# bowang-lab/BioReason

Hardware: AMD Instinct MI355X
Metric: GRPO samples/sec (NT-500M+Qwen3-1.7B, DNA 2x1024, prompt 2180, gen 256) (higher is better)
Workload: dtype bf16

## Files before the change

bioreason_amd/csrc/k_misc.hip:

```cpp
#include "bra_device.h"
#include "bra_api_internal.h"

namespace bra {

template <int HD>
__global__ __launch_bounds__(256) void head_transpose_kernel(const bf16_t* x, long sb, long ss, long sh, bf16_t* xt,
                                                             long t_sb, long t_sh, long pitch, int S) {
    constexpr int LD = HD + 2;
    __shared__ bf16_t tile[64 * LD];
    const int tid = (int)threadIdx.x;
    const int s0 = (int)blockIdx.x * 64, h = (int)blockIdx.y, b = (int)blockIdx.z;
    const bf16_t* xp = x + b * sb + h * sh;
    constexpr int CH = HD / 8;
    for (int q = tid; q < 64 * CH; q += 256) {
        const int r = q / CH, c = q % CH;
        const int s = s0 + r;
        u32x4 v = {0u, 0u, 0u, 0u};
        if (s < S) v = ld16(xp + (long)s * ss + c * 8);
        uint32_t* tp = reinterpret_cast<uint32_t*>(&tile[r * LD + c * 8]);
        tp[0] = v.x; tp[1] = v.y; tp[2] = v.z; tp[3] = v.w;
    }
    __syncthreads();
    bf16_t* op = xt + b * t_sb + h * t_sh;
    for (int q = tid; q < HD * 8; q += 256) {
        const int d = q >> 3, c = q & 7;
        uint32_t w[4];
#pragma unroll
        for (int i = 0; i < 4; ++i) {
            const uint32_t lo = tile[(c * 8 + 2 * i) * LD + d], hi = tile[(c * 8 + 2 * i + 1) * LD + d];
            w[i] = lo | (hi << 16);
        }
        u32x4 v = {w[0], w[1], w[2], w[3]};
        st16(op + (long)d * pitch + s0 + c * 8, v);
    }
}

__global__ __launch_bounds__(256) void attn_delta_kernel(const bf16_t* dout, long do_sb, long do_ss, long do_sh,
                                                         const bf16_t* o, long o_sb, long o_ss, long o_sh,
                                                         float* delta, int B, int S, int H, int hd) {
    const int lpr = hd / 8;
    const long total = (long)B * H * S * lpr;
    const long idx = (long)blockIdx.x * 256 + threadIdx.x;
    const bool live = idx < total;
    const long cl = live ? idx : total - 1;
    const int c = (int)(cl % lpr);
    const long row = cl / lpr;
    const int s = (int)(row % S);
    const int h = (int)((row / S) % H);
    const int b = (int)(row / ((long)S * H));
    float f[8], g[8];
    unpack8(ld16(dout + b * do_sb + (long)s * do_ss + h * do_sh + c * 8), f);
    unpack8(ld16(o + b * o_sb + (long)s * o_ss + h * o_sh + c * 8), g);
    float acc = 0.f;
#pragma unroll
    for (int i = 0; i < 8; ++i) acc += f[i] * g[i];
    for (int m = lpr >> 1; m >= 1; m >>= 1) acc += wave_shfl_xor(acc, m);
    if (live && c == 0) delta[row] = acc;
}

__global__ __launch_bounds__(1024) void dna_scatter_plan_kernel(const int* ids, int ntok, int dna_id,
                                                                const uint8_t* dna_mask, int nseq, int Sd,
                                                                const int* seq_order, int* tok_src, int* counts) {
    __shared__ int feat_base[1025];
    __shared__ int wsum[16];
    __shared__ int carry;
    const int tid = (int)threadIdx.x, lane = tid & 63, wave = tid >> 6;
    for (int k = wave; k < nseq; k += 16) {
        const int seq = seq_order[k];
        int cnt = 0;
        for (int p = lane; p < Sd; p += 64) cnt += dna_mask[(long)seq * Sd + p] ? 1 : 0;
        for (int m = 32; m >= 1; m >>= 1) cnt += wave_shfl_xor_i(cnt, m);
        if (lane == 0) feat_base[k + 1] = cnt;
// ... 244 lines not shown
    else if (hd == 32) BRA_LAUNCH((head_transpose_kernel<32>), grid, dim3(256), 0, stream, (const bf16_t*)x, sb, ss, sh, (bf16_t*)xt, t_sb, t_sh, pitch, S);
    else return BRA_ERR_UNSUPPORTED;
    return BRA_LAUNCH_STATUS();
}

extern "C" int bra_attn_delta(const void* dout, long do_sb, long do_ss, long do_sh, const void* o, long o_sb,
                              long o_ss, long o_sh, float* delta, int B, int S, int H, int hd, void* stream) {
    if (B <= 0 || S <= 0 || H <= 0) return 0;
    if (!dout || !o || !delta || (hd != 32 && hd != 64 && hd != 128)) return BRA_ERR_ARG;
    const long total = (long)B * H * S * (hd / 8);
    BRA_LAUNCH(attn_delta_kernel, dim3((unsigned)((total + 255) / 256)), dim3(256), 0, stream, (const bf16_t*)dout,
               do_sb, do_ss, do_sh, (const bf16_t*)o, o_sb, o_ss, o_sh, delta, B, S, H, hd);
    return BRA_LAUNCH_STATUS();
}

extern "C" int bra_dna_scatter_plan(const int* ids, int ntok, int dna_id, const void* dna_mask, int nseq, int Sd,
                                    const int* seq_order, int* tok_src, int* counts, void* stream) {
    if (!ids || !tok_src || !counts || ntok < 0 || nseq < 0 || nseq > 1024) return BRA_ERR_ARG;
    if (nseq > 0 && (!dna_mask || !seq_order || Sd <= 0)) return BRA_ERR_ARG;
    BRA_LAUNCH(dna_scatter_plan_kernel, dim3(1), dim3(1024), 0, stream, ids, ntok, dna_id, (const uint8_t*)dna_mask,
               nseq, Sd, seq_order, tok_src, counts);
    return BRA_LAUNCH_STATUS();
}

extern "C" int bra_embed_scatter_fwd(const int* ids, const int* tok_src, const void* E, long lde, const void* dna,
                                     long ldd, void* out, long ldo, int ntok, int H, void* stream) {
    if (ntok == 0) return 0;
    if (!ids || !E || !out || H % 8 || lde % 8 || ldo % 8 || (tok_src && (!dna || ldd % 8))) return BRA_ERR_ARG;
    BRA_LAUNCH(embed_scatter_fwd_kernel, dim3(ew_grid((long)ntok * (H / 8))), dim3(256), 0, stream, ids, tok_src,
               (const bf16_t*)E, lde, (const bf16_t*)dna, ldd, (bf16_t*)out, ldo, ntok, H);
// ... 157 lines not shown
```

bioreason_amd/csrc/k_norm.hip:

```cpp
#include "bra_device.h"
#include "bra_api_internal.h"

namespace bra {

__global__ __launch_bounds__(256) void rmsnorm_fwd_kernel(const bf16_t* x, long ldx, const bf16_t* w, bf16_t* y,
                                                          long ldy, float* rstd_out, int rows, int cols, float eps) {
    const int row = (int)blockIdx.x * 4 + (int)(threadIdx.x >> 6);
    const int lane = lane_id();
    const bool live = row < rows;
    const bf16_t* xr = x + (long)(live ? row : 0) * ldx;
    float ss = 0.f;
    for (int c = lane * 8; c < cols; c += 512) {
        float f[8];
        unpack8(ld16(xr + c), f);
#pragma unroll
        for (int i = 0; i < 8; ++i) ss += f[i] * f[i];
    }
    ss = wave_sum<64>(ss);
    const float rstd = rsqrtf(ss / (float)cols + eps);
    if (!live) return;
    if (rstd_out && lane == 0) rstd_out[row] = rstd;
    bf16_t* yr = y + (long)row * ldy;
    for (int c = lane * 8; c < cols; c += 512) {
        float f[8], g[8];
// ... 224 lines not shown
    float w1 = 1.f, w2 = 1.f;
    if (nw) { w1 = bf2f(nw[d]); w2 = bf2f(nw[d + half]); dot = w1 * g1 * x1 + w2 * g2 * x2; }
    for (int m = half >> 1; m >= 1; m >>= 1) { ss += wave_shfl_xor(ss, m); dot += wave_shfl_xor(dot, m); }
    if (nw) {
        const float rstd = rsqrtf(ss / (float)a.hd + a.eps);
        const float cm = dot * rstd / (float)a.hd;
        g1 = rstd * (w1 * g1 - x1 * rstd * cm);
        g2 = rstd * (w2 * g2 - x2 * rstd * cm);
    }
    if (!live) return;
    bf16_t* dst = a.dqkv + (long)t * a.lddqkv + (long)h * a.hd;
    dst[d] = f2bf(g1);
    dst[d + half] = f2bf(g2);
}

template <int HD>
__global__ __launch_bounds__(256) void qk_norm_rope_fwd_vec_kernel(RopeArgs a) {
    constexpr int LPH = HD / 8, HALF = HD / 2;
    const int H = a.Hq + 2 * a.Hkv;
    const long nhead = (long)a.T * H;
    const long gl = (long)blockIdx.x * 256 + threadIdx.x;
    const long hidx = gl / LPH;
    const int j = (int)(gl % LPH);
    const bool live = hidx < nhead;
    const long hc = live ? hidx : nhead - 1;
    const int h = (int)(hc % H);
    const int t = (int)(hc / H);
    const bool is_q = h < a.Hq, is_k = !is_q && h < a.Hq + a.Hkv;
    const bool upper = j >= LPH / 2;
    const int dh = (j & (LPH / 2 - 1)) * 8;
    float x[8];
    unpack8(ld16(a.qkv + (long)t * a.ldqkv + (long)h * HD + j * 8), x);
    const bf16_t* nw = is_q ? a.qw : (is_k ? a.kw : nullptr);
    u32x4 nwv = {0u, 0u, 0u, 0u};
    if (nw) nwv = ld16(nw + j * 8);
    f32x4 c0 = {1.f, 1.f, 1.f, 1.f}, c1 = c0, s0 = {0.f, 0.f, 0.f, 0.f}, s1 = s0;
    if (is_q || is_k) {
        const int p = a.pos[t];
        const float* cp = a.cosT + (long)p * HALF + dh;
        const float* sp = a.sinT + (long)p * HALF + dh;
        c0 = *reinterpret_cast<const f32x4*>(cp); c1 = *reinterpret_cast<const f32x4*>(cp + 4);
        s0 = *reinterpret_cast<const f32x4*>(sp); s1 = *reinterpret_cast<const f32x4*>(sp + 4);
    }
    float ss = 0.f;
#pragma unroll
    for (int i = 0; i < 8; ++i) ss += x[i] * x[i];
#pragma unroll
    for (int m = LPH >> 1; m >= 1; m >>= 1) ss += wave_shfl_xor(ss, m);
    if (nw) {
        const float rstd = rsqrtf(ss / (float)HD + a.eps);
        float w[8];
        unpack8(nwv, w);
#pragma unroll
        for (int i = 0; i < 8; ++i) x[i] = round_bf(w[i] * round_bf(x[i] * rstd));
    }
    if (is_q && a.qscale != 1.f) {
#pragma unroll
        for (int i = 0; i < 8; ++i) x[i] = round_bf(x[i] * a.qscale);
    }
    float o[8];
#pragma unroll
    for (int i = 0; i < 8; ++i) {
        const float other = wave_shfl_xor(x[i], LPH / 2);
        const float c = i < 4 ? c0[i & 3] : c1[i & 3], sn = i < 4 ? s0[i & 3] : s1[i & 3];
        o[i] = (is_q || is_k) ? (upper ? x[i] * c + other * sn : x[i] * c - other * sn) : x[i];
    }
    if (!live) return;
    const int b = t / a.S, sidx = t % a.S;
    bf16_t* dst;
    if (is_q) dst = a.q + b * a.q_sb + sidx * a.q_ss + (long)h * a.q_sh;
    else if (is_k) dst = a.k + b * a.k_sb + (sidx + a.s_off) * a.k_ss + (long)(h - a.Hq) * a.k_sh;
    else dst = a.v + b * a.v_sb + (sidx + a.s_off) * a.v_ss + (long)(h - a.Hq - a.Hkv) * a.v_sh;
    st16(dst + j * 8, pack8(o));
}

template <int HD>
__global__ __launch_bounds__(256) void qk_norm_rope_bwd_vec_kernel(RopeBwdArgs a) {
    constexpr int LPH = HD / 8, HALF = HD / 2;
    const int H = a.Hq + 2 * a.Hkv;
    const long nhead = (long)a.T * H;
    const long gl = (long)blockIdx.x * 256 + threadIdx.x;
    const long hidx = gl / LPH;
    const int j = (int)(gl % LPH);
    const bool live = hidx < nhead;
    const long hc = live ? hidx : nhead - 1;
    const int h = (int)(hc % H);
    const int t = (int)(hc / H);
    const bool is_q = h < a.Hq, is_k = !is_q && h < a.Hq + a.Hkv;
// ... 113 lines not shown
                  hd, eps, qscale, (bf16_t*)q, q_sb, q_ss, q_sh, (bf16_t*)k, k_sb, k_ss, k_sh, (bf16_t*)v, v_sb,
                  v_ss, v_sh, s_off};
    const long total = (long)T * (Hq + 2 * Hkv) * (hd / 2);
    const bool vec = (hd == 128 || hd == 64) && ldqkv % 8 == 0 && !((q_sb | q_ss | q_sh | k_sb | k_ss | k_sh | v_sb | v_ss | v_sh) & 7);
    if (vec) {
        const long lanes = (long)T * (Hq + 2 * Hkv) * (hd / 8);
        const dim3 grid((unsigned)((lanes + 255) / 256));
        if (hd == 128) BRA_LAUNCH((qk_norm_rope_fwd_vec_kernel<128>), grid, dim3(256), 0, stream, a);
        else BRA_LAUNCH((qk_norm_rope_fwd_vec_kernel<64>), grid, dim3(256), 0, stream, a);
        return BRA_LAUNCH_STATUS();
    }
    BRA_LAUNCH(qk_norm_rope_fwd_kernel, dim3((unsigned)((total + 255) / 256)), dim3(256), 0, stream, a);
    return BRA_LAUNCH_STATUS();
}

extern "C" int bra_qk_norm_rope_bwd(const void* qkv, long ldqkv, const void* qw, const void* kw, const float* cosT,
                                    const float* sinT, const int* pos, int T, int S, int Hq, int Hkv, int hd,
                                    float eps, float qscale, const void* dq, long q_sb, long q_ss, long q_sh,
                                    const void* dk, long k_sb, long k_ss, long k_sh, const void* dv, long v_sb,
                                    long v_ss, long v_sh, void* dqkv, long lddqkv, void* stream) {
    if (T == 0) return 0;
    if (!qkv || !cosT || !sinT || !pos || !dq || !dk || !dv || !dqkv || S <= 0 || T % S) return BRA_ERR_ARG;
    if (!pow2(hd) || hd < 2 || hd > 128) return BRA_ERR_UNSUPPORTED;
    RopeBwdArgs a = {(const bf16_t*)qkv, ldqkv, (const bf16_t*)qw, (const bf16_t*)kw, cosT, sinT, pos, T, S, Hq,
                     Hkv, hd, eps, qscale, (const bf16_t*)dq, q_sb, q_ss, q_sh, (const bf16_t*)dk, k_sb, k_ss, k_sh,
                     (const bf16_t*)dv, v_sb, v_ss, v_sh, (bf16_t*)dqkv, lddqkv};
    const long total = (long)T * (Hq + 2 * Hkv) * (hd / 2);
    const bool vec = (hd == 128 || hd == 64) && ldqkv % 8 == 0 && lddqkv % 8 == 0 &&
                     !((q_sb | q_ss | q_sh | k_sb | k_ss | k_sh | v_sb | v_ss | v_sh) & 7);
    if (vec) {
// ... 10 lines not shown
```

bioreason_amd/engine.py:

```python
from __future__ import annotations

import math
from dataclasses import dataclass, field
from typing import Dict, List, Optional, Tuple

import torch

from . import ops
from .arena import TrainableArena

BF16 = torch.bfloat16


def rope_tables(npos: int, hd: int, theta: float, device, round_bf16: bool = True) -> Tuple[torch.Tensor, torch.Tensor]:
    inv = 1.0 / (theta ** (torch.arange(0, hd, 2, dtype=torch.float32) / hd))
    fr = torch.arange(npos, dtype=torch.float32)[:, None] * inv[None, :]
    c, s = fr.cos(), fr.sin()
    if round_bf16:
        c, s = c.to(BF16).float(), s.to(BF16).float()
    return c.contiguous().to(device), s.contiguous().to(device)


class LoraGroup:

# ... 196 lines not shown

    def _layer_fwd_fp8(self, li: int, x: torch.Tensor, m: SeqMeta, kv_out, R):
        L = self.layers[li]
        B, S, T = m.B, m.S, m.B * m.S
        cosT, sinT = self.rope(m.max_pos or m.S)
        xq, xs = ops.quant_rows_fp8(x, rms_eps=self.eps)
        qkv = ops.gemm_fp8_nt(xq, xs, R["Wqkv"][0], R["Wqkv"][1])
        q = torch.empty((B, S, self.Hq, self.hd), dtype=BF16, device=x.device)
        if kv_out is None:
            k = torch.empty((B, S, self.Hkv, self.hd), dtype=BF16, device=x.device)
            v = torch.empty((B, S, self.Hkv, self.hd), dtype=BF16, device=x.device)
            s_off = 0
        else:
            kc, vc, s_off = kv_out[:3]
            k, v = kc.permute(0, 2, 1, 3), vc.permute(0, 2, 1, 3)
        ops.qk_norm_rope_fwd(qkv, L.qn, L.kn, cosT, sinT, m.pos, S, self.Hq, self.Hkv, self.hd, self.eps, 1.0, q, k, v, s_off)
        if kv_out is not None:
            k, v = k[:, :s_off + S], v[:, :s_off + S]
        vt = ops.head_transpose(v)
        if kv_out is not None and len(kv_out) > 3 and kv_out[3] is not None:
            kv_out[3].append(vt)
        o, _ = ops.attn_fwd(q, k, vt, m.kmask, True, self.scale, need_lse=False)
        oq, os_ = ops.quant_rows_fp8(o.view(T, self.Nq))
        h = ops.gemm_fp8_nt(oq, os_, R["Wo"][0], R["Wo"][1], res=x)
        hq, hs = ops.quant_rows_fp8(h, rms_eps=self.eps)
        gu = ops.gemm_fp8_nt(hq, hs, R["Wgu"][0], R["Wgu"][1])
        aq, as_ = ops.swiglu_quant_fp8(gu)
        return ops.gemm_fp8_nt(aq, as_, R["Wd"][0], R["Wd"][1], res=h)

    def layer_fwd(self, li: int, x: torch.Tensor, m: SeqMeta, save: bool, kv_out=None):
        w8 = getattr(self, "_fp8", None)
        if w8 is not None and not save:
            return self._layer_fwd_fp8(li, x, m, kv_out, w8[li]), None
        L = self.layers[li]
        B, S, T = m.B, m.S, m.B * m.S
        cosT, sinT = self.rope(m.max_pos or m.S)
        xn = ops.rmsnorm_fwd(x, L.ln1, self.eps)
        qkv, t1 = self._lora_fwd(xn, L.Wqkv, L.lora["qkv"], m.lora_on, drop=self._drop(m, li, "qkv"))
        q = torch.empty((B, S, self.Hq, self.hd), dtype=BF16, device=x.device)
        if kv_out is None:
            k = torch.empty((B, S, self.Hkv, self.hd), dtype=BF16, device=x.device)
            v = torch.empty((B, S, self.Hkv, self.hd), dtype=BF16, device=x.device)
            s_off = 0
        else:
            kc, vc, s_off = kv_out[:3]
            k, v = kc.permute(0, 2, 1, 3), vc.permute(0, 2, 1, 3)
        ops.qk_norm_rope_fwd(qkv, L.qn, L.kn, cosT, sinT, m.pos, S, self.Hq, self.Hkv, self.hd, self.eps, 1.0, q, k, v, s_off)
        if kv_out is not None:
            k, v = k[:, :s_off + S], v[:, :s_off + S]
        vt = ops.head_transpose(v)
        if kv_out is not None and len(kv_out) > 3 and kv_out[3] is not None:
            kv_out[3].append(vt)
        o, lse = ops.attn_fwd(q, k, vt, m.kmask, True, self.scale, need_lse=save)
        o2 = o.view(T, self.Nq)
        h, t2 = self._lora_fwd(o2, L.Wo, L.lora["o"], m.lora_on, res=x, drop=self._drop(m, li, "o"))
        hn = ops.rmsnorm_fwd(h, L.ln2, self.eps)
        gu = t3 = act = None
        if not save and FUSE_SWIGLU:
            G3, d3 = L.lora["gu"], self._drop(m, li, "gu")
            if G3 is not None and m.lora_on:
                t3 = ops.lora_down_drop(hn, G3.A, G3.scaling, d3[0], d3[1], d3[2]) if d3 is not None else self._down(hn, G3.A, G3.scaling, len(G3.n_sizes) * G3.r)
                act = ops.gemm_swiglu(hn, L.Wgu, a2=t3, b2=G3.B)
            else:
                act = ops.gemm_swiglu(hn, L.Wgu)
        if act is None:
            if t3 is not None:
                gu = ops.gemm_nt(hn, L.Wgu, a2=t3, b2=L.lora["gu"].B)
            else:
                gu, t3 = self._lora_fwd(hn, L.Wgu, L.lora["gu"], m.lora_on, drop=self._drop(m, li, "gu"))
            act = ops.swiglu_fwd(gu)
        y, t4 = self._lora_fwd(act, L.Wd, L.lora["d"], m.lora_on, res=h, drop=self._drop(m, li, "d"))
        saved = (x, xn, t1, qkv, q, k, v, o, lse, t2, h, hn, t3, gu, act, t4) if save else None
        return y, saved

    def layer_bwd(self, li: int, dy: torch.Tensor, saved, m: SeqMeta, prefix: int = 0, extra_dkv=None):
        L = self.layers[li]
        (x, xn, t1, qkv, q, k, v, o, lse, t2, h, hn, t3, gu, act, t4) = saved
        B, S, T = m.B, m.S, m.B * m.S
        cosT, sinT = self.rope(m.max_pos or m.S)
        on = m.lora_on
        dact = self._lora_bwd(dy, L.WdT, L.lora["d"], on, act, t4, drop=self._drop(m, li, "d"))
        dgu = ops.swiglu_bwd(gu, dact)
        dhn = self._lora_bwd(dgu, L.WguT, L.lora["gu"], on, hn, t3, drop=self._drop(m, li, "gu"))
        dh = ops.rmsnorm_bwd(dhn, h, L.ln2, self.eps, dres=dy)
        do = self._lora_bwd(dh, L.WoT, L.lora["o"], on, o.view(T, self.Nq), t2, drop=self._drop(m, li, "o"))
        dq, dk, dv = ops.attn_bwd(q, k, v, o, do.view(B, S, self.Hq, self.hd), lse, m.kmask, True, self.scale)
        pre = None
        if prefix > 0:
            pre = (dk[:, :prefix], dv[:, :prefix])
            dk, dv = dk[:, prefix:], dv[:, prefix:]
        if extra_dkv is not None:
            dk = ops.group_sum(extra_dkv[0], extra_dkv[2], add=dk)
            dv = ops.group_sum(extra_dkv[1], extra_dkv[2], add=dv)
        dqkv = ops.qk_norm_rope_bwd(qkv, L.qn, L.kn, cosT, sinT, m.pos, S, self.Hq, self.Hkv, self.hd, self.eps, 1.0, dq, dk, dv)
        dxn = self._lora_bwd(dqkv, L.WqkvT, L.lora["qkv"], on, xn, t1, drop=self._drop(m, li, "qkv"))
        dx = ops.rmsnorm_bwd(dxn, x, L.ln1, self.eps, dres=dh)
        return (dx, pre) if prefix > 0 else dx

    def forward_hidden(self, x: torch.Tensor, m: SeqMeta, save: bool):
        tape = []
        for li in range(self.L):
# ... 124 lines not shown
        n, S = ids32.shape
        T = n * S
        dev = ids32.device
        cosT, sinT = self.rope(S)
        pos = torch.arange(S, dtype=torch.int32, device=dev).repeat(n)
        x = torch.empty((T, self.H), dtype=BF16, device=dev)
        zero_row = torch.zeros((1, self.H), dtype=BF16, device=dev)
        tok_src = (mask_u8.reshape(-1).to(torch.int32) - 1).clamp_(max=0).neg_().sub_(1)
        ops.embed_scatter_fwd(ids32.reshape(-1), tok_src, self.E, zero_row, x)
        for L in self.layers:
            xn = ops.layernorm_fwd(x, L.ln1_w, L.ln1_b, self.eps)
            qkv = ops.gemm_nt(xn, L.Wqkv, bias=L.bqkv)
            q = torch.empty((n, S, self.nh, self.hd), dtype=BF16, device=dev)
            k = torch.empty_like(q)
            v = torch.empty_like(q)
            ops.qk_norm_rope_fwd(qkv, None, None, cosT, sinT, pos, S, self.nh, self.nh, self.hd, 0.0, self.hd ** -0.5, q, k, v, 0)
            vt = ops.head_transpose(v)
            o, _ = ops.attn_fwd(q, k, vt, mask_u8, False, 1.0, need_lse=False)
            x = ops.gemm_nt(o.view(T, self.H), L.Wo, bias=L.bo, res=x)
            xn = ops.layernorm_fwd(x, L.ln2_w, L.ln2_b, self.eps)
            act = ops.gemm_swiglu(xn, L.Wup) if FUSE_SWIGLU else None
            if act is None:
                act = ops.swiglu_fwd(ops.gemm_nt(xn, L.Wup))
            x = ops.gemm_nt(act, L.Wdown, res=x)
        return ops.layernorm_fwd(x, self.lnf_w, self.lnf_b, self.eps)
```

bioreason_amd/ops.py:

```python
from __future__ import annotations

import math
import os
from typing import Optional, Tuple

import torch

from ._lib import current_stream, get_lib

BF16 = torch.bfloat16


def _ld(t: torch.Tensor) -> int:
    assert t.stride(-1) == 1, "last dim must be contiguous"
    return t.stride(-2) if t.dim() >= 2 else t.shape[-1]


def _rows(t: torch.Tensor) -> int:
    return t.numel() // t.shape[-1]


def _as2d(t: torch.Tensor) -> torch.Tensor:
    return t.reshape(-1, t.shape[-1]) if t.dim() != 2 else t

# ... 233 lines not shown
    get_lib().call("bra_swiglu_bwd", gu2, _ld(gu2), d2, _ld(d2), dgu, _ld(dgu), gu2.shape[0], F, current_stream(gu))
    return dgu


def _bsh_strides(t: torch.Tensor) -> Tuple[int, int, int]:
    assert t.dim() == 4 and t.stride(3) == 1
    return t.stride(0), t.stride(1), t.stride(2)


def qk_norm_rope_fwd(qkv, qw, kw, cosT, sinT, pos, S, Hq, Hkv, hd, eps, qscale, q, k, v, s_off=0):
    T = qkv.shape[0]
    get_lib().call("bra_qk_norm_rope_fwd", qkv, _ld(qkv), qw, kw, cosT, sinT, pos, T, S, Hq, Hkv, hd, eps, qscale,
                   q, *_bsh_strides(q), k, *_bsh_strides(k), v, *_bsh_strides(v), s_off, current_stream(qkv))


def qk_norm_rope_bwd(qkv, qw, kw, cosT, sinT, pos, S, Hq, Hkv, hd, eps, qscale, dq, dk, dv):
    T = qkv.shape[0]
    dqkv = torch.empty_like(qkv)
    get_lib().call("bra_qk_norm_rope_bwd", qkv, _ld(qkv), qw, kw, cosT, sinT, pos, T, S, Hq, Hkv, hd, eps, qscale,
                   dq, *_bsh_strides(dq), dk, *_bsh_strides(dk), dv, *_bsh_strides(dv), dqkv, _ld(dqkv), current_stream(qkv))
    return dqkv


def pad64(n: int) -> int:
    return (n + 63) // 64 * 64


def head_transpose(x: torch.Tensor) -> torch.Tensor:
    B, S, H, hd = x.shape
    out = torch.empty((B, H, hd, pad64(S)), dtype=BF16, device=x.device)
# ... 33 lines not shown
    if wgs >= 200:
        return 1
    return max(1, min(4, (300 + wgs // 2) // wgs))


def attn_bwd_split_parts(B: int, Hq: int, Hkv: int, Sq: int, Sk: int, hd: int, causal: bool):
    ns_dq = attn_fwd_split_parts(B, Hq, Sq, Sk, hd, causal)
    ns_kv = 1
    if ATTN_SPLIT and hd >= 64 and Sq >= 1024 and Sk > 128:
        wgs = ((Sk + 255) // 256) * Hkv * B
        if wgs < 200:
            ns_kv = max(1, min(4, (300 + wgs // 2) // wgs))
    return ns_dq, ns_kv


def attn_bwd(q, k, v, o, dout, lse, kmask, causal: bool, scale: float, q_off: Optional[int] = None, nsplit=None):
    B, Sq, Hq, hd = q.shape
    Sk, Hkv = k.shape[1], k.shape[2]
    if q_off is None:
        q_off = Sk - Sq
    lib = get_lib()
    st = current_stream(q)
    delta = torch.empty((B, Hq, Sq), dtype=torch.float32, device=q.device)
    lib.call("bra_attn_delta", dout, *_bsh_strides(dout), o, *_bsh_strides(o), delta, B, Sq, Hq, hd, st)
    kt = head_transpose(k)
    qt = head_transpose(q)
    dot = head_transpose(dout)
    dq = torch.empty((B, Sq, Hq, hd), dtype=BF16, device=q.device)
    dk = torch.empty((B, Sk, Hkv, hd), dtype=BF16, device=q.device)
    dv = torch.empty((B, Sk, Hkv, hd), dtype=BF16, device=q.device)
    ns_dq, ns_kv = attn_bwd_split_parts(B, Hq, Hkv, Sq, Sk, hd, causal) if nsplit is None else nsplit
    if ns_dq > 1 or ns_kv > 1:
        part_dq = torch.empty((B, Hq, ns_dq, Sq, hd), dtype=torch.float32, device=q.device) if ns_dq > 1 else None
        part_dk = torch.empty((B, Hkv, ns_kv, Sk, hd), dtype=torch.float32, device=q.device) if ns_kv > 1 else None
        part_dv = torch.empty((B, Hkv, ns_kv, Sk, hd), dtype=torch.float32, device=q.device) if ns_kv > 1 else None
        lib.call("bra_attn_bwd_split", q, *_bsh_strides(q), k, *_bsh_strides(k), v, *_bsh_strides(v), dout, *_bsh_strides(dout),
                 kt, kt.stride(0), kt.stride(1), kt.stride(2), qt, qt.stride(0), qt.stride(1), qt.stride(2),
                 dot, dot.stride(0), dot.stride(1), dot.stride(2), lse, delta, kmask,
                 dq, *_bsh_strides(dq), dk, *_bsh_strides(dk), dv, *_bsh_strides(dv),
                 B, Hq, Hkv, Sq, Sk, hd, int(causal), q_off, scale, ns_dq, part_dq, ns_kv, part_dk, part_dv, st)
        return dq, dk, dv
    lib.call("bra_attn_bwd", q, *_bsh_strides(q), k, *_bsh_strides(k), v, *_bsh_strides(v), dout, *_bsh_strides(dout),
# ... 349 lines not shown
```

include/bioreason_hip.h:

```cpp
#ifndef BIOREASON_HIP_H
#define BIOREASON_HIP_H
#ifdef __cplusplus
extern "C" {
#endif

#define BRA_ERR_ARG (-1)
#define BRA_ERR_UNSUPPORTED (-2)

int bra_gemm_bf16_nt(const void* A, long lda, const void* B, long ldb, const void* A2, long lda2, const void* B2,
                     long ldb2, int K2, void* C, long ldc, int M, int N, int K, float alpha, const void* bias,
                     const void* res, long ldres, int out_f32, int accumulate, void* stream);

int bra_gemm_bf16_nt_splitk(const void* A, long lda, const void* B, long ldb, void* C, long ldc, int M, int N, int K,
                            float alpha, int split_k, void* stream);

int bra_wgrad_tn(const void* Y, long ldy, const void* T, long ldt, float* C, long c_sn, long c_sr, int M, int N, int R,
                 float alpha, int m_chunk, void* stream);

int bra_lora_down_splitk_plan(int M, int K);
int bra_lora_down_drop(const void* x, long ldx, const void* A, long lda, void* t, long ldt, int M, int K, int R, float alpha,
                       float p, unsigned s0, unsigned s1, unsigned s2, unsigned s3, int r, int nt, float* part, int ksplit,
                       void* stream);
int bra_lora_up_drop(const void* dts, long ldd, const void* AT, long ldat, void* out, long ldo, int M, int K, int R, float p,
                     unsigned s0, unsigned s1, unsigned s2, unsigned s3, int r, int nt, void* stream);
// ... 10 lines not shown
                       const float* lse, const float* coef, void* dlogits, long ldd, void* stream);

int bra_rmsnorm_fwd(const void* x, long ldx, const void* w, void* y, long ldy, float* rstd, int rows, int cols,
                    float eps, void* stream);
int bra_rmsnorm_bwd(const void* dy, long lddy, const void* x, long ldx, const void* w, const void* dres, long lddres,
                    void* dx, long lddx, int rows, int cols, float eps, void* stream);
int bra_layernorm_fwd(const void* x, long ldx, const void* w, const void* b, void* y, long ldy, int rows, int cols,
                      float eps, void* stream);
int bra_swiglu_fwd(const void* gu, long ldgu, void* act, long ldact, int rows, int F, void* stream);
int bra_swiglu_bwd(const void* gu, long ldgu, const void* dact, long lddact, void* dgu, long lddgu, int rows, int F,
                   void* stream);
int bra_qk_norm_rope_fwd(const void* qkv, long ldqkv, const void* qw, const void* kw, const float* cosT,
                         const float* sinT, const int* pos, int T, int S, int Hq, int Hkv, int hd, float eps,
                         float qscale, void* q, long q_sb, long q_ss, long q_sh, void* k, long k_sb, long k_ss,
                         long k_sh, void* v, long v_sb, long v_ss, long v_sh, int s_off, void* stream);
int bra_qk_norm_rope_bwd(const void* qkv, long ldqkv, const void* qw, const void* kw, const float* cosT,
                         const float* sinT, const int* pos, int T, int S, int Hq, int Hkv, int hd, float eps,
                         float qscale, const void* dq, long q_sb, long q_ss, long q_sh, const void* dk, long k_sb,
                         long k_ss, long k_sh, const void* dv, long v_sb, long v_ss, long v_sh, void* dqkv,
                         long lddqkv, void* stream);

int bra_attn_fwd(const void* q, long q_sb, long q_ss, long q_sh, const void* k, long k_sb, long k_ss, long k_sh,
                 const void* vt, long vt_sb, long vt_sh, long vt_sd, void* o, long o_sb, long o_ss, long o_sh,
                 float* lse, const void* kmask, int B, int Hq, int Hkv, int Sq, int Sk, int hd, int causal,
                 int q_off, float scale, void* stream);
int bra_attn_fwd_split(const void* q, long q_sb, long q_ss, long q_sh, const void* k, long k_sb, long k_ss, long k_sh,
                       const void* vt, long vt_sb, long vt_sh, long vt_sd, void* o, long o_sb, long o_ss, long o_sh,
                       float* lse, const void* kmask, int B, int Hq, int Hkv, int Sq, int Sk, int hd, int causal,
                       int q_off, float scale, int nsplit, float* part_o, float* part_ml, void* stream);
int bra_attn_bwd(const void* q, long q_sb, long q_ss, long q_sh, const void* k, long k_sb, long k_ss, long k_sh,
// ... 78 lines not shown
                     const int* pos, const float* rope_rows, const void* kp, long kp_sr, long kp_sh, long kp_ss,
                     const void* vtp, long vt_sr, long vt_sh, long vt_sd, const void* pmask, void* kc, void* vct, long cp,
                     float* part_o, float* part_ml, int nslot, void* o, long ldo, int R, int copies,
                     int Hq, int Hkv, int hd, int P, int C, int t, float eps, float scale, const int* t_dev, void* stream);
int bra_qwen_decode_step_one(const void* layers_host, int L, int R, int copies, int H, int Hq, int Hkv, int hd, int F,
                             int P, long vt_pitch, int C, long cp, int V, float eps, float scale, const void* E,
                             const void* norm_w, const float* cosT, const float* sinT, const int* tok, const int* pos,
                             const void* pmask, int t, const int* t_dev, int embed_done, void* x, void* qkv, void* o, void* h,
                             void* act, float* ss_ws, int nss, float* part_o, float* part_ml, int nslot, float* logits,
                             void* stream);

int bra_head_transpose(const void* x, long sb, long ss, long sh, void* xt, long t_sb, long t_sh, long pitch, int B,
                       int S, int H, int hd, void* stream);
int bra_attn_delta(const void* dout, long do_sb, long do_ss, long do_sh, const void* o, long o_sb, long o_ss,
                   long o_sh, float* delta, int B, int S, int H, int hd, void* stream);
int bra_dna_scatter_plan(const int* ids, int ntok, int dna_id, const void* dna_mask, int nseq, int Sd,
                         const int* seq_order, int* tok_src, int* counts, void* stream);
int bra_embed_scatter_fwd(const int* ids, const int* tok_src, const void* E, long lde, const void* dna, long ldd,
                          void* out, long ldo, int ntok, int H, void* stream);
int bra_embed_scatter_bwd(const int* tok_src, const void* dout, long ldo, void* ddna, long ldd, int ntok, int H,
                          void* stream);
int bra_gather_rows(const int* rows, const void* x, long ldx, void* out, long ldo, int n, int H, void* stream);
int bra_scatter_rows(const int* rows, const void* x, long ldx, void* out, long ldo, int n, int H, void* stream);
int bra_transpose2d(const void* in, long ldi, void* out, long ldo, int rows, int cols, void* stream);
int bra_colsum(const void* x, long ldx, float* out, int rows, int cols, void* stream);
int bra_pack_desc_size(void);
int bra_pack_params(const void* descs_dev, int ndesc, long max_elems, void* stream);
int bra_vec_sum(const float* x, long n, float scale, float* out, void* stream);
int bra_cast_grad(const void* src, void* dst, long n, int to_f32, void* stream);
int bra_sumsq(const float* g, const void* mask, long n, float* out, float* ws, void* stream);
// ... 50 lines not shown
```

Measured before the change: 19.59.

## Fuse head transposes into QK-norm/RoPE forward and attention delta kernels

Adds a QK-norm+RoPE forward kernel that writes the head-transposed V, and optionally Q and K, straight from its LDS tile. This removes the separate head_transpose launches in the forward pass and in attention backward; the transposed Q and K are saved for backward. The attention delta computation is fused with the transpose of dout into one kernel. Each of these removes an extra read of the activations and one launch per layer. In exchange, memory for saved activations grows, and the dot-product ordering is pinned to keep numerics bitwise stable.

```diff
diff --git a/bioreason_amd/csrc/bra_transpose.h b/bioreason_amd/csrc/bra_transpose.h
--- /dev/null
+++ b/bioreason_amd/csrc/bra_transpose.h
@@ -0,0 +1,31 @@
+#pragma once
+#include "bra_device.h"
+
+namespace bra {
+
+constexpr int kTRows = 64;
+template <int HD> constexpr int ttile_elems() { return kTRows * (HD + 2); }
+
+template <int HD>
+__device__ __forceinline__ void ttile_put(bf16_t* tile, int r, int c, const u32x4& v) {
+    uint32_t* tp = reinterpret_cast<uint32_t*>(&tile[r * (HD + 2) + c * 8]);
+    tp[0] = v.x; tp[1] = v.y; tp[2] = v.z; tp[3] = v.w;
+}
+
+template <int HD>
+__device__ __forceinline__ void ttile_store(const bf16_t* tile, bf16_t* op, long pitch, int s0, int tid) {
+    constexpr int LD = HD + 2;
+    for (int q = tid; q < HD * 8; q += 256) {
+        const int d = q >> 3, c = q & 7;
+        uint32_t w[4];
+#pragma unroll
+        for (int i = 0; i < 4; ++i) {
+            const uint32_t lo = tile[(c * 8 + 2 * i) * LD + d], hi = tile[(c * 8 + 2 * i + 1) * LD + d];
+            w[i] = lo | (hi << 16);
+        }
+        u32x4 v = {w[0], w[1], w[2], w[3]};
+        st16(op + (long)d * pitch + s0 + c * 8, v);
+    }
+}
+
+}
diff --git a/bioreason_amd/csrc/k_misc.hip b/bioreason_amd/csrc/k_misc.hip
--- a/bioreason_amd/csrc/k_misc.hip
+++ b/bioreason_amd/csrc/k_misc.hip
@@ -1,13 +1,13 @@
 #include "bra_device.h"
 #include "bra_api_internal.h"
+#include "bra_transpose.h"
 
 namespace bra {
 
 template <int HD>
 __global__ __launch_bounds__(256) void head_transpose_kernel(const bf16_t* x, long sb, long ss, long sh, bf16_t* xt,
                                                              long t_sb, long t_sh, long pitch, int S) {
-    constexpr int LD = HD + 2;
-    __shared__ bf16_t tile[64 * LD];
+    __shared__ bf16_t tile[ttile_elems<HD>()];
     const int tid = (int)threadIdx.x;
     const int s0 = (int)blockIdx.x * 64, h = (int)blockIdx.y, b = (int)blockIdx.z;
     const bf16_t* xp = x + b * sb + h * sh;
@@ -17,22 +17,18 @@
         const int s = s0 + r;
         u32x4 v = {0u, 0u, 0u, 0u};
         if (s < S) v = ld16(xp + (long)s * ss + c * 8);
-        uint32_t* tp = reinterpret_cast<uint32_t*>(&tile[r * LD + c * 8]);
-        tp[0] = v.x; tp[1] = v.y; tp[2] = v.z; tp[3] = v.w;
-    }
-    __syncthreads();
-    bf16_t* op = xt + b * t_sb + h * t_sh;
-    for (int q = tid; q < HD * 8; q += 256) {
-        const int d = q >> 3, c = q & 7;
-        uint32_t w[4];
-#pragma unroll
-        for (int i = 0; i < 4; ++i) {
-            const uint32_t lo = tile[(c * 8 + 2 * i) * LD + d], hi = tile[(c * 8 + 2 * i + 1) * LD + d];
-            w[i] = lo | (hi << 16);
-        }
-        u32x4 v = {w[0], w[1], w[2], w[3]};
-        st16(op + (long)d * pitch + s0 + c * 8, v);
-    }
+        ttile_put<HD>(tile, r, c, v);
+    }
+    __syncthreads();
+    ttile_store<HD>(tile, xt + b * t_sb + h * t_sh, pitch, s0, tid);
+}
+
+__device__ __forceinline__ float delta_dot8(const float* f, const float* g) {
+#pragma clang fp contract(off)
+#pragma clang fp reassociate(off)
+    const float a = __builtin_fmaf(f[1], g[1], __builtin_fmaf(f[4], g[4], __builtin_fmaf(f[2], g[2], f[6] * g[6])));
+    const float b = __builtin_fmaf(f[0], g[0], __builtin_fmaf(f[5], g[5], __builtin_fmaf(f[3], g[3], f[7] * g[7])));
+    return a + b;
 }
 
 __global__ __launch_bounds__(256) void attn_delta_kernel(const bf16_t* dout, long do_sb, long do_ss, long do_sh,
@@ -51,11 +47,40 @@
     float f[8], g[8];
     unpack8(ld16(dout + b * do_sb + (long)s * do_ss + h * do_sh + c * 8), f);
     unpack8(ld16(o + b * o_sb + (long)s * o_ss + h * o_sh + c * 8), g);
-    float acc = 0.f;
-#pragma unroll
-    for (int i = 0; i < 8; ++i) acc += f[i] * g[i];
+    float acc = delta_dot8(f, g);
     for (int m = lpr >> 1; m >= 1; m >>= 1) acc += wave_shfl_xor(acc, m);
     if (live && c == 0) delta[row] = acc;
+}
+
+template <int HD>
+__global__ __launch_bounds__(256) void attn_delta_t_kernel(const bf16_t* dout, long do_sb, long do_ss, long do_sh,
+                                                           const bf16_t* o, long o_sb, long o_ss, long o_sh, float* delta,
+                                                           bf16_t* dot, long t_sb, long t_sh, long pitch, int S, int H) {
+    __shared__ bf16_t tile[ttile_elems<HD>()];
+    constexpr int CH = HD / 8;
+    const int tid = (int)threadIdx.x;
+    const int s0 = (int)blockIdx.x * 64, h = (int)blockIdx.y, b = (int)blockIdx.z;
+    const bf16_t* dp = dout + b * do_sb + h * do_sh;
+    const bf16_t* op = o + b * o_sb + h * o_sh;
+#pragma unroll
+    for (int it = 0; it < 64 * CH / 256; ++it) {
+        const int q = tid + it * 256;
+        const int r = q / CH, c = q % CH;
+        const int s = s0 + r;
+        const bool live = s < S;
+        u32x4 dv = {0u, 0u, 0u, 0u}, ov = dv;
+        if (live) { dv = ld16(dp + (long)s * do_ss + c * 8); ov = ld16(op + (long)s * o_ss + c * 8); }
+        float f[8], g[8];
+        unpack8(dv, f);
+        unpack8(ov, g);
+        float acc = delta_dot8(f, g);
+#pragma unroll
+        for (int m = CH >> 1; m >= 1; m >>= 1) acc += wave_shfl_xor(acc, m);
+        if (live && c == 0) delta[((long)b * H + h) * S + s] = acc;
+        ttile_put<HD>(tile, r, c, dv);
+    }
+    __syncthreads();
+    ttile_store<HD>(tile, dot + b * t_sb + h * t_sh, pitch, s0, tid);
 }
 
 __global__ __launch_bounds__(1024) void dna_scatter_plan_kernel(const int* ids, int ntok, int dna_id,
@@ -330,6 +355,24 @@
     return BRA_LAUNCH_STATUS();
 }
 
+extern "C" int bra_attn_delta_t(const void* dout, long do_sb, long do_ss, long do_sh, const void* o, long o_sb,
+                                long o_ss, long o_sh, float* delta, void* dot, long t_sb, long t_sh, long pitch, int B,
+                                int S, int H, int hd, void* stream) {
+    if (B <= 0 || S <= 0 || H <= 0) return 0;
+    if (!dout || !o || !delta || !dot || pitch % 64 || pitch < ((S + 63) / 64) * 64) return BRA_ERR_ARG;
+    if ((do_sb | do_ss | do_sh | o_sb | o_ss | o_sh | t_sb | t_sh) & 7) return BRA_ERR_ARG;
+    const dim3 grid((S + 63) / 64, H, B);
+#define BRA_DELTA_T(HD)                                                                                                    \
+    BRA_LAUNCH((attn_delta_t_kernel<HD>), grid, dim3(256), 0, stream, (const bf16_t*)dout, do_sb, do_ss, do_sh,            \
+               (const bf16_t*)o, o_sb, o_ss, o_sh, delta, (bf16_t*)dot, t_sb, t_sh, pitch, S, H)
+    if (hd == 128) BRA_DELTA_T(128);
+    else if (hd == 64) BRA_DELTA_T(64);
+    else if (hd == 32) BRA_DELTA_T(32);
+    else return BRA_ERR_UNSUPPORTED;
+#undef BRA_DELTA_T
+    return BRA_LAUNCH_STATUS();
+}
+
 extern "C" int bra_dna_scatter_plan(const int* ids, int ntok, int dna_id, const void* dna_mask, int nseq, int Sd,
                                     const int* seq_order, int* tok_src, int* counts, void* stream) {
     if (!ids || !tok_src || !counts || ntok < 0 || nseq < 0 || nseq > 1024) return BRA_ERR_ARG;
diff --git a/bioreason_amd/csrc/k_norm.hip b/bioreason_amd/csrc/k_norm.hip
--- a/bioreason_amd/csrc/k_norm.hip
+++ b/bioreason_amd/csrc/k_norm.hip
@@ -1,5 +1,6 @@
 #include "bra_device.h"
 #include "bra_api_internal.h"
+#include "bra_transpose.h"
 
 namespace bra {
 
@@ -262,23 +263,21 @@
     dst[d + half] = f2bf(g2);
 }
 
+
+#ifdef BRA_EMU
+__device__ __forceinline__ float opaque_f(float x) { return x; }
+#else
+__device__ __forceinline__ float opaque_f(float x) { asm volatile("" : "+v"(x)); return x; }
+#endif
+
 template <int HD>
-__global__ __launch_bounds__(256) void qk_norm_rope_fwd_vec_kernel(RopeArgs a) {
+__device__ __forceinline__ void rope_fwd_lane(const RopeArgs& a, int t, int h, int j, float* x, float* o) {
+#pragma clang fp contract(off)
+#pragma clang fp reassociate(off)
     constexpr int LPH = HD / 8, HALF = HD / 2;
-    const int H = a.Hq + 2 * a.Hkv;
-    const long nhead = (long)a.T * H;
-    const long gl = (long)blockIdx.x * 256 + threadIdx.x;
-    const long hidx = gl / LPH;
-    const int j = (int)(gl % LPH);
-    const bool live = hidx < nhead;
-    const long hc = live ? hidx : nhead - 1;
-    const int h = (int)(hc % H);
-    const int t = (int)(hc / H);
     const bool is_q = h < a.Hq, is_k = !is_q && h < a.Hq + a.Hkv;
     const bool upper = j >= LPH / 2;
     const int dh = (j & (LPH / 2 - 1)) * 8;
-    float x[8];
-    unpack8(ld16(a.qkv + (long)t * a.ldqkv + (long)h * HD + j * 8), x);
     const bf16_t* nw = is_q ? a.qw : (is_k ? a.kw : nullptr);
     u32x4 nwv = {0u, 0u, 0u, 0u};
     if (nw) nwv = ld16(nw + j * 8);
@@ -290,13 +289,13 @@
         c0 = *reinterpret_cast<const f32x4*>(cp); c1 = *reinterpret_cast<const f32x4*>(cp + 4);
         s0 = *reinterpret_cast<const f32x4*>(sp); s1 = *reinterpret_cast<const f32x4*>(sp + 4);
     }
-    float ss = 0.f;
-#pragma unroll
-    for (int i = 0; i < 8; ++i) ss += x[i] * x[i];
+    float ss = x[0] * x[0];
+#pragma unroll
+    for (int i = 1; i < 8; ++i) ss = __builtin_fmaf(x[i], x[i], ss);
 #pragma unroll
     for (int m = LPH >> 1; m >= 1; m >>= 1) ss += wave_shfl_xor(ss, m);
     if (nw) {
-        const float rstd = rsqrtf(ss / (float)HD + a.eps);
+        const float rstd = rsqrtf(__builtin_fmaf(ss, 1.f / (float)HD, a.eps));
         float w[8];
         unpack8(nwv, w);
 #pragma unroll
@@ -306,20 +305,85 @@
 #pragma unroll
         for (int i = 0; i < 8; ++i) x[i] = round_bf(x[i] * a.qscale);
     }
-    float o[8];
 #pragma unroll
     for (int i = 0; i < 8; ++i) {
         const float other = wave_shfl_xor(x[i], LPH / 2);
         const float c = i < 4 ? c0[i & 3] : c1[i & 3], sn = i < 4 ? s0[i & 3] : s1[i & 3];
-        o[i] = (is_q || is_k) ? (upper ? x[i] * c + other * sn : x[i] * c - other * sn) : x[i];
-    }
+        const float xc = opaque_f(x[i] * c), os = opaque_f(other * sn);
+        o[i] = (is_q || is_k) ? (upper ? xc + os : xc - os) : x[i];
+    }
+}
+
+__device__ __forceinline__ bf16_t* rope_dst_row(const RopeArgs& a, int h, int b, int row) {
+    if (h < a.Hq) return a.q + b * a.q_sb + row * a.q_ss + (long)h * a.q_sh;
+    if (h < a.Hq + a.Hkv) return a.k + b * a.k_sb + row * a.k_ss + (long)(h - a.Hq) * a.k_sh;
+    return a.v + b * a.v_sb + row * a.v_ss + (long)(h - a.Hq - a.Hkv) * a.v_sh;
+}
+
+template <int HD>
+__global__ __launch_bounds__(256) void qk_norm_rope_fwd_vec_kernel(RopeArgs a) {
+    constexpr int LPH = HD / 8;
+    const int H = a.Hq + 2 * a.Hkv;
+    const long nhead = (long)a.T * H;
+    const long gl = (long)blockIdx.x * 256 + threadIdx.x;
+    const long hidx = gl / LPH;
+    const int j = (int)(gl % LPH);
+    const bool live = hidx < nhead;
+    const long hc = live ? hidx : nhead - 1;
+    const int h = (int)(hc % H);
+    const int t = (int)(hc / H);
+    float x[8], o[8];
+    unpack8(ld16(a.qkv + (long)t * a.ldqkv + (long)h * HD + j * 8), x);
+    rope_fwd_lane<HD>(a, t, h, j, x, o);
     if (!live) return;
     const int b = t / a.S, sidx = t % a.S;
-    bf16_t* dst;
-    if (is_q) dst = a.q + b * a.q_sb + sidx * a.q_ss + (long)h * a.q_sh;
-    else if (is_k) dst = a.k + b * a.k_sb + (sidx + a.s_off) * a.k_ss + (long)(h - a.Hq) * a.k_sh;
-    else dst = a.v + b * a.v_sb + (sidx + a.s_off) * a.v_ss + (long)(h - a.Hq - a.Hkv) * a.v_sh;
-    st16(dst + j * 8, pack8(o));
+    st16(rope_dst_row(a, h, b, sidx + (h < a.Hq ? 0 : a.s_off)) + j * 8, pack8(o));
+}
+
+struct RopeTArgs {
+    RopeArgs r;
+    bf16_t* qt; long qt_sb, qt_sh, qt_pitch;
+    bf16_t* kt; long kt_sb, kt_sh, kt_pitch;
+    bf16_t* vt; long vt_sb, vt_sh, vt_pitch;
+};
+
+template <int HD>
+__global__ __launch_bounds__(256) void qk_norm_rope_fwd_t_kernel(RopeTArgs ta) {
+    __shared__ bf16_t tile[ttile_elems<HD>()];
+    constexpr int CH = HD / 8;
+    const RopeArgs& a = ta.r;
+    const int tid = (int)threadIdx.x;
+    const int s0 = (int)blockIdx.x * 64, h = (int)blockIdx.y, b = (int)blockIdx.z;
+    const bool is_q = h < a.Hq, is_k = !is_q && h < a.Hq + a.Hkv;
+    const int off = is_q ? 0 : a.s_off;
+    const int n = off + a.S;
+    bf16_t* xt = is_q ? ta.qt : (is_k ? ta.kt : ta.vt);
+    if (s0 >= n || (!xt && s0 + 64 <= off)) return;
+#pragma unroll
+    for (int it = 0; it < 64 * CH / 256; ++it) {
+        const int q = tid + it * 256;
+        const int r = q / CH, j = q % CH;
+        const int row = s0 + r;
+        const bool fresh = row >= off && row < n;
+        const int t = b * a.S + (fresh ? row - off : 0);
+        u32x4 v = ld16(a.qkv + (long)t * a.ldqkv + (long)h * HD + j * 8);
+        if (is_q || is_k) {
+            float x[8], o[8];
+            unpack8(v, x);
+            rope_fwd_lane<HD>(a, t, h, j, x, o);
+            v = pack8(o);
+        }
+        bf16_t* dst = rope_dst_row(a, h, b, row < n ? row : 0) + j * 8;
+        if (fresh) st16(dst, v);
+        else if (xt && row < off) v = ld16(dst);
+        else v = u32x4{0u, 0u, 0u, 0u};
+        if (xt) ttile_put<HD>(tile, r, j, v);
+    }
+    if (!xt) return;
+    __syncthreads();
+    const int ht = is_q ? h : (is_k ? h - a.Hq : h - a.Hq - a.Hkv);
+    const long t_sb = is_q ? ta.qt_sb : (is_k ? ta.kt_sb : ta.vt_sb), t_sh = is_q ? ta.qt_sh : (is_k ? ta.kt_sh : ta.vt_sh);
+    ttile_store<HD>(tile, xt + b * t_sb + ht * t_sh, is_q ? ta.qt_pitch : (is_k ? ta.kt_pitch : ta.vt_pitch), s0, tid);
 }
 
 template <int HD>
@@ -463,6 +527,33 @@
     return BRA_LAUNCH_STATUS();
 }
 
+extern "C" int bra_qk_norm_rope_fwd_t(const void* qkv, long ldqkv, const void* qw, const void* kw, const float* cosT,
+                                      const float* sinT, const int* pos, int T, int S, int Hq, int Hkv, int hd,
+                                      float eps, float qscale, void* q, long q_sb, long q_ss, long q_sh, void* k,
+                                      long k_sb, long k_ss, long k_sh, void* v, long v_sb, long v_ss, long v_sh,
+                                      int s_off, void* qt, long qt_sb, long qt_sh, long qt_pitch, void* kt, long kt_sb,
+                                      long kt_sh, long kt_pitch, void* vt, long vt_sb, long vt_sh, long vt_pitch,
+                                      void* stream) {
+    if (T == 0) return 0;
+    if (!qkv || !cosT || !sinT || !pos || !q || !k || !v || !vt || S <= 0 || T % S || s_off < 0 || Hq <= 0 || Hkv <= 0)
+        return BRA_ERR_ARG;
+    if (hd != 128 && hd != 64) return BRA_ERR_UNSUPPORTED;
+    if (ldqkv % 8 || ((q_sb | q_ss | q_sh | k_sb | k_ss | k_sh | v_sb | v_ss | v_sh) & 7)) return BRA_ERR_UNSUPPORTED;
+    const long pad_q = ((long)S + 63) / 64 * 64, pad_kv = ((long)s_off + S + 63) / 64 * 64;
+    if (qt && (qt_pitch % 64 || qt_pitch < pad_q || ((qt_sb | qt_sh) & 7))) return BRA_ERR_ARG;
+    if (kt && (kt_pitch % 64 || kt_pitch < pad_kv || ((kt_sb | kt_sh) & 7))) return BRA_ERR_ARG;
+    if (vt_pitch % 64 || vt_pitch < pad_kv || ((vt_sb | vt_sh) & 7)) return BRA_ERR_ARG;
+    RopeTArgs a = {{(const bf16_t*)qkv, ldqkv, (const bf16_t*)qw, (const bf16_t*)kw, cosT, sinT, pos, T, S, Hq, Hkv,
+                    hd, eps, qscale, (bf16_t*)q, q_sb, q_ss, q_sh, (bf16_t*)k, k_sb, k_ss, k_sh, (bf16_t*)v, v_sb,
+                    v_ss, v_sh, s_off},
+                   (bf16_t*)qt, qt_sb, qt_sh, qt_pitch, (bf16_t*)kt, kt_sb, kt_sh, kt_pitch, (bf16_t*)vt, vt_sb, vt_sh,
+                   vt_pitch};
+    const dim3 grid((unsigned)(pad_kv / 64), (unsigned)(Hq + 2 * Hkv), (unsigned)(T / S));
+    if (hd == 128) BRA_LAUNCH((qk_norm_rope_fwd_t_kernel<128>), grid, dim3(256), 0, stream, a);
+    else BRA_LAUNCH((qk_norm_rope_fwd_t_kernel<64>), grid, dim3(256), 0, stream, a);
+    return BRA_LAUNCH_STATUS();
+}
+
 extern "C" int bra_qk_norm_rope_bwd(const void* qkv, long ldqkv, const void* qw, const void* kw, const float* cosT,
                                     const float* sinT, const int* pos, int T, int S, int Hq, int Hkv, int hd,
                                     float eps, float qscale, const void* dq, long q_sb, long q_ss, long q_sh,
diff --git a/bioreason_amd/engine.py b/bioreason_amd/engine.py
--- a/bioreason_amd/engine.py
+++ b/bioreason_amd/engine.py
@@ -234,10 +234,9 @@
         else:
             kc, vc, s_off = kv_out[:3]
             k, v = kc.permute(0, 2, 1, 3), vc.permute(0, 2, 1, 3)
-        ops.qk_norm_rope_fwd(qkv, L.qn, L.kn, cosT, sinT, m.pos, S, self.Hq, self.Hkv, self.hd, self.eps, 1.0, q, k, v, s_off)
+        vt, _, _ = ops.qk_norm_rope_fwd_t(qkv, L.qn, L.kn, cosT, sinT, m.pos, S, self.Hq, self.Hkv, self.hd, self.eps, 1.0, q, k, v, s_off)
         if kv_out is not None:
             k, v = k[:, :s_off + S], v[:, :s_off + S]
-        vt = ops.head_transpose(v)
         if kv_out is not None and len(kv_out) > 3 and kv_out[3] is not None:
             kv_out[3].append(vt)
         o, _ = ops.attn_fwd(q, k, vt, m.kmask, True, self.scale, need_lse=False)
@@ -265,10 +264,10 @@
         else:
             kc, vc, s_off = kv_out[:3]
             k, v = kc.permute(0, 2, 1, 3), vc.permute(0, 2, 1, 3)
-        ops.qk_norm_rope_fwd(qkv, L.qn, L.kn, cosT, sinT, m.pos, S, self.Hq, self.Hkv, self.hd, self.eps, 1.0, q, k, v, s_off)
+        vt, qt, kt = ops.qk_norm_rope_fwd_t(qkv, L.qn, L.kn, cosT, sinT, m.pos, S, self.Hq, self.Hkv, self.hd, self.eps, 1.0, q, k, v,
+                                            s_off, want_qk_t=save)
         if kv_out is not None:
             k, v = k[:, :s_off + S], v[:, :s_off + S]
-        vt = ops.head_transpose(v)
         if kv_out is not None and len(kv_out) > 3 and kv_out[3] is not None:
             kv_out[3].append(vt)
         o, lse = ops.attn_fwd(q, k, vt, m.kmask, True, self.scale, need_lse=save)
@@ -290,12 +289,12 @@
                 gu, t3 = self._lora_fwd(hn, L.Wgu, L.lora["gu"], m.lora_on, drop=self._drop(m, li, "gu"))
             act = ops.swiglu_fwd(gu)
         y, t4 = self._lora_fwd(act, L.Wd, L.lora["d"], m.lora_on, res=h, drop=self._drop(m, li, "d"))
-        saved = (x, xn, t1, qkv, q, k, v, o, lse, t2, h, hn, t3, gu, act, t4) if save else None
+        saved = (x, xn, t1, qkv, q, k, v, o, lse, t2, h, hn, t3, gu, act, t4, qt, kt) if save else None
         return y, saved
 
     def layer_bwd(self, li: int, dy: torch.Tensor, saved, m: SeqMeta, prefix: int = 0, extra_dkv=None):
         L = self.layers[li]
-        (x, xn, t1, qkv, q, k, v, o, lse, t2, h, hn, t3, gu, act, t4) = saved
+        (x, xn, t1, qkv, q, k, v, o, lse, t2, h, hn, t3, gu, act, t4, qt, kt) = saved
         B, S, T = m.B, m.S, m.B * m.S
         cosT, sinT = self.rope(m.max_pos or m.S)
         on = m.lora_on
@@ -304,7 +303,7 @@
         dhn = self._lora_bwd(dgu, L.WguT, L.lora["gu"], on, hn, t3, drop=self._drop(m, li, "gu"))
         dh = ops.rmsnorm_bwd(dhn, h, L.ln2, self.eps, dres=dy)
         do = self._lora_bwd(dh, L.WoT, L.lora["o"], on, o.view(T, self.Nq), t2, drop=self._drop(m, li, "o"))
-        dq, dk, dv = ops.attn_bwd(q, k, v, o, do.view(B, S, self.Hq, self.hd), lse, m.kmask, True, self.scale)
+        dq, dk, dv = ops.attn_bwd(q, k, v, o, do.view(B, S, self.Hq, self.hd), lse, m.kmask, True, self.scale, qt=qt, kt=kt)
         pre = None
         if prefix > 0:
             pre = (dk[:, :prefix], dv[:, :prefix])
@@ -459,8 +458,7 @@
             q = torch.empty((n, S, self.nh, self.hd), dtype=BF16, device=dev)
             k = torch.empty_like(q)
             v = torch.empty_like(q)
-            ops.qk_norm_rope_fwd(qkv, None, None, cosT, sinT, pos, S, self.nh, self.nh, self.hd, 0.0, self.hd ** -0.5, q, k, v, 0)
-            vt = ops.head_transpose(v)
+            vt, _, _ = ops.qk_norm_rope_fwd_t(qkv, None, None, cosT, sinT, pos, S, self.nh, self.nh, self.hd, 0.0, self.hd ** -0.5, q, k, v, 0)
             o, _ = ops.attn_fwd(q, k, vt, mask_u8, False, 1.0, need_lse=False)
             x = ops.gemm_nt(o.view(T, self.H), L.Wo, bias=L.bo, res=x)
             xn = ops.layernorm_fwd(x, L.ln2_w, L.ln2_b, self.eps)
diff --git a/bioreason_amd/ops.py b/bioreason_amd/ops.py
--- a/bioreason_amd/ops.py
+++ b/bioreason_amd/ops.py
@@ -271,6 +271,24 @@
                    q, *_bsh_strides(q), k, *_bsh_strides(k), v, *_bsh_strides(v), s_off, current_stream(qkv))
 
 
+def qk_norm_rope_fwd_t(qkv, qw, kw, cosT, sinT, pos, S, Hq, Hkv, hd, eps, qscale, q, k, v, s_off=0, want_qk_t=False):
+    T = qkv.shape[0]
+    B, n = T // S, s_off + S
+    if hd not in (64, 128):
+        qk_norm_rope_fwd(qkv, qw, kw, cosT, sinT, pos, S, Hq, Hkv, hd, eps, qscale, q, k, v, s_off)
+        vt = head_transpose(v[:, :n])
+        return (vt, head_transpose(q), head_transpose(k[:, :n])) if want_qk_t else (vt, None, None)
+    vt = torch.empty((B, Hkv, hd, pad64(n)), dtype=BF16, device=qkv.device)
+    qt = torch.empty((B, Hq, hd, pad64(S)), dtype=BF16, device=qkv.device) if want_qk_t else None
+    kt = torch.empty((B, Hkv, hd, pad64(n)), dtype=BF16, device=qkv.device) if want_qk_t else None
+    tq = (qt, qt.stride(0), qt.stride(1), qt.stride(2)) if want_qk_t else (None, 0, 0, 0)
+    tk = (kt, kt.stride(0), kt.stride(1), kt.stride(2)) if want_qk_t else (None, 0, 0, 0)
+    get_lib().call("bra_qk_norm_rope_fwd_t", qkv, _ld(qkv), qw, kw, cosT, sinT, pos, T, S, Hq, Hkv, hd, eps, qscale,
+                   q, *_bsh_strides(q), k, *_bsh_strides(k), v, *_bsh_strides(v), s_off, *tq, *tk,
+                   vt, vt.stride(0), vt.stride(1), vt.stride(2), current_stream(qkv))
+    return vt, qt, kt
+
+
 def qk_norm_rope_bwd(qkv, qw, kw, cosT, sinT, pos, S, Hq, Hkv, hd, eps, qscale, dq, dk, dv):
     T = qkv.shape[0]
     dqkv = torch.empty_like(qkv)
@@ -334,18 +352,27 @@
     return ns_dq, ns_kv
 
 
-def attn_bwd(q, k, v, o, dout, lse, kmask, causal: bool, scale: float, q_off: Optional[int] = None, nsplit=None):
+def attn_delta_t(dout, o):
+    B, Sq, Hq, hd = dout.shape
+    delta = torch.empty((B, Hq, Sq), dtype=torch.float32, device=dout.device)
+    dot = torch.empty((B, Hq, hd, pad64(Sq)), dtype=BF16, device=dout.device)
+    get_lib().call("bra_attn_delta_t", dout, *_bsh_strides(dout), o, *_bsh_strides(o), delta, dot, dot.stride(0), dot.stride(1),
+                   dot.stride(2), B, Sq, Hq, hd, current_stream(dout))
+    return delta, dot
+
+
+def attn_bwd(q, k, v, o, dout, lse, kmask, causal: bool, scale: float, q_off: Optional[int] = None, nsplit=None, qt=None, kt=None):
     B, Sq, Hq, hd = q.shape
     Sk, Hkv = k.shape[1], k.shape[2]
     if q_off is None:
         q_off = Sk - Sq
     lib = get_lib()
     st = current_stream(q)
-    delta = torch.empty((B, Hq, Sq), dtype=torch.float32, device=q.device)
-    lib.call("bra_attn_delta", dout, *_bsh_strides(dout), o, *_bsh_strides(o), delta, B, Sq, Hq, hd, st)
-    kt = head_transpose(k)
-    qt = head_transpose(q)
-    dot = head_transpose(dout)
+    delta, dot = attn_delta_t(dout, o)
+    if kt is None:
+        kt = head_transpose(k)
+    if qt is None:
+        qt = head_transpose(q)
     dq = torch.empty((B, Sq, Hq, hd), dtype=BF16, device=q.device)
     dk = torch.empty((B, Sk, Hkv, hd), dtype=BF16, device=q.device)
     dv = torch.empty((B, Sk, Hkv, hd), dtype=BF16, device=q.device)
diff --git a/include/bioreason_hip.h b/include/bioreason_hip.h
--- a/include/bioreason_hip.h
+++ b/include/bioreason_hip.h
@@ -48,6 +48,12 @@
                          const float* sinT, const int* pos, int T, int S, int Hq, int Hkv, int hd, float eps,
                          float qscale, void* q, long q_sb, long q_ss, long q_sh, void* k, long k_sb, long k_ss,
                          long k_sh, void* v, long v_sb, long v_ss, long v_sh, int s_off, void* stream);
+int bra_qk_norm_rope_fwd_t(const void* qkv, long ldqkv, const void* qw, const void* kw, const float* cosT,
+                           const float* sinT, const int* pos, int T, int S, int Hq, int Hkv, int hd, float eps,
+                           float qscale, void* q, long q_sb, long q_ss, long q_sh, void* k, long k_sb, long k_ss,
+                           long k_sh, void* v, long v_sb, long v_ss, long v_sh, int s_off, void* qt, long qt_sb,
+                           long qt_sh, long qt_pitch, void* kt, long kt_sb, long kt_sh, long kt_pitch, void* vt,
+                           long vt_sb, long vt_sh, long vt_pitch, void* stream);
 int bra_qk_norm_rope_bwd(const void* qkv, long ldqkv, const void* qw, const void* kw, const float* cosT,
                          const float* sinT, const int* pos, int T, int S, int Hq, int Hkv, int hd, float eps,
                          float qscale, const void* dq, long q_sb, long q_ss, long q_sh, const void* dk, long k_sb,
@@ -156,6 +162,9 @@
                        int S, int H, int hd, void* stream);
 int bra_attn_delta(const void* dout, long do_sb, long do_ss, long do_sh, const void* o, long o_sb, long o_ss,
                    long o_sh, float* delta, int B, int S, int H, int hd, void* stream);
+int bra_attn_delta_t(const void* dout, long do_sb, long do_ss, long do_sh, const void* o, long o_sb, long o_ss,
+                     long o_sh, float* delta, void* dot, long t_sb, long t_sh, long pitch, int B, int S, int H, int hd,
+                     void* stream);
 int bra_dna_scatter_plan(const int* ids, int ntok, int dna_id, const void* dna_mask, int nseq, int Sd,
                          const int* seq_order, int* tok_src, int* counts, void* stream);
 int bra_embed_scatter_fwd(const int* ids, const int* tok_src, const void* E, long lde, const void* dna, long ldd,
```

Result: no change. 19.64 (median of 3 runs) (+0.3%).
